# JingInAI/Quantize

Measured on AMD Instinct MI355X. Metric: quant-conv2d images/sec at batch 256 (ResNet-50, W8A8), higher is better.
Workload: dtype int8

## Files before the change

quantize_amd/capi.py:

```python
import contextlib
import ctypes
import os

from . import loader

_lib = None

QE_OK = 0
QE_ERR_UNSUPPORTED = 7
DTYPES = {"uint8": 0, "int8": 1, "int16": 2, "int32": 3, "int64": 4,
          "float16": 5, "float32": 6, "float64": 7}

ACTS = {None: 0, "none": 0, "gelu": 1}


class QeConvShape(ctypes.Structure):
    _fields_ = [(n, ctypes.c_int32) for n in ("N", "IC", "H", "W", "OC", "KH", "KW", "stride", "padding")]


class QeQParam(ctypes.Structure):
    _fields_ = [("data", ctypes.c_void_p), ("n_bits", ctypes.c_int32), ("sign", ctypes.c_int32),
                ("scale", ctypes.c_void_p), ("zero", ctypes.c_void_p), ("n_param", ctypes.c_int32)]


# ... 20 lines not shown
    "qe_tpack": (_i32, [_vp, _i32, _i64, _i32, _i32, _vp, _vp, _vp]),
    "qe_tunpack": (_i32, [_vp, _i64, _i32, _i32, _vp, _vp]),
    "qe_quantize_pack": (_i32, [_vp, _i64, _vp, _vp, _i32, _i64, _f32, _f32, _i32, _i32, _vp, _vp, _vp]),
    "qe_quantize_pack_act": (_i32, [_vp, _i64, _i32, _vp, _vp, _i32, _i64, _f32, _f32, _i32, _i32, _vp, _vp, _vp, _vp]),
    "qe_quantize_patchify": (_i32, [_vp, _i32, _i32, _i32, _i32, _i32, _vp, _vp, _i32, _f32, _f32, _i32, _i32, _vp, _vp, _vp]),
    "qe_global_avgpool": (_i32, [_vp, _i64, _i32, _vp, _vp]),
    "qe_maxpool2d_codes": (_i32, [_vp, _i32, _i32, _i32, _i32, _i32, _i32, _i32, _vp, _vp]),
    "qe_quantconv2d_path": (_i32, [_ps, _pq, _pq]),
    "qe_quantconv2d_workspace_bytes": (_sz, [_ps, _i32, _i32]),
    "qe_quantconv2d": (_i32, [_pq, _pq, _vp, _ps, _vp, _vp, _sz, _vp]),
    "qe_conv_prepared_bytes": (_sz, [_ps, _i32, _i32]),
    "qe_conv_prepared_layout": (ctypes.c_uint64, [_ps, _i32, _i32]),
    "qe_conv_prepare": (_i32, [_pq, _vp, _ps, _i32, _vp, _sz, _vp]),
    "qe_quantconv2d_prepared_workspace_bytes": (_sz, [_ps, _i32, _i32]),
    "qe_quantconv2d_prepared": (_i32, [_pq, _pq, _vp, _ps, _vp, _sz, _vp, _vp, _sz, _vp]),
    "qe_quantconv2d_requant_path": (_i32, [_ps, _pq, _pq, _pr]),
    "qe_quantconv2d_requant_workspace_bytes": (_sz, [_ps, _pq, _pq, _pr]),
    "qe_quantconv2d_requant_prepared": (_i32, [_pq, _pq, _vp, _ps, _vp, _sz, _pr, _vp, _vp, _vp, _sz, _vp]),
    "qe_quantconv2d_residual_path": (_i32, [_ps, _pq, _pq, _pr]),
    "qe_quantconv2d_residual_workspace_bytes": (_sz, [_ps, _pq, _pq, _pr]),
    "qe_quantconv2d_residual_prepared": (_i32, [_pq, _pq, _vp, _ps, _vp, _sz, _vp, _vp, _pr, _vp, _vp, _vp, _sz, _vp]),
    "qe_quantconv2d_float_input": (_i32, [_vp, _pq, _vp, _ps, _vp, _vp]),
    "qe_quantconv2d_float_input_path": (_i32, [_ps, _pq]),
    "qe_quantconv2d_float_input_workspace_bytes": (_sz, [_ps, _i32]),
    "qe_quantconv2d_float_input_ws": (_i32, [_vp, _pq, _vp, _ps, _vp, _vp, _sz, _vp]),
    "qe_conv_f32_prepare": (_i32, [_pq, _vp, _ps, _vp, _sz, _vp]),
    "qe_quantconv2d_float_input_prepared": (_i32, [_vp, _pq, _vp, _ps, _vp, _sz, _vp, _vp]),
    "qe_quantlinear": (_i32, [_pq, _pq, _vp, _i64, _i32, _i32, _vp, _vp]),
    "qe_quantlinear_path": (_i32, [_pq, _pq, _i64, _i32, _i32]),
    "qe_quantlinear_form": (_i32, [_pq, _pq, _i64, _i32, _i32, _i32]),
    "qe_quantlinear_float_input": (_i32, [_vp, _pq, _vp, _i64, _i32, _i32, _vp, _vp]),
    "qe_quantlinear_float_input_path": (_i32, [_vp, _pq, _i64, _i32, _i32]),
    "qe_quantlinear_requant_path": (_i32, [_pq, _pq, _i64, _i32, _i32, _pr, _vp]),
    "qe_quantlinear_requant_workspace_bytes": (_sz, [_pq, _pq, _i64, _i32, _i32, _pr, _vp]),
    "qe_quantlinear_requant": (_i32, [_pq, _pq, _vp, _i64, _i32, _i32, _i32, _pr, _vp, _vp, _vp, _sz, _vp]),
    "qe_quantlinear_residual_path": (_i32, [_pq, _pq, _i64, _i32, _i32]),
    "qe_quantlinear_residual_workspace_bytes": (_sz, [_pq, _pq, _i64, _i32, _i32]),
    "qe_quantlinear_residual": (_i32, [_pq, _pq, _vp, _i64, _i32, _i32, _vp, _vp, _vp, _sz, _vp]),
    "qe_quantlinear_float_input_residual_path": (_i32, [_vp, _pq, _i64, _i32, _i32]),
    "qe_quantlinear_float_input_residual_workspace_bytes": (_sz, [_vp, _pq, _i64, _i32, _i32]),
    "qe_quantlinear_float_input_residual": (_i32, [_vp, _pq, _vp, _i64, _i32, _i32, _vp, _vp, _vp, _sz, _vp]),
    "qe_layernorm_quantize_pack_path": (_i32, [_i64, _i32, _i32, _pr, _ppc]),
    "qe_layernorm_quantize_pack_workspace_bytes": (_sz, [_i64, _i32, _i32, _pr, _ppc, _vp]),
    "qe_layernorm_quantize_pack": (_i32, [_vp, _i64, _i32, _vp, _vp, _f32, _i32, _pr, _ppc, _vp, _vp, _vp, _sz, _vp]),
    "qe_attention_path": (_i32, [_i32, _i32, _i32, _i32]),
    "qe_attention": (_i32, _attn + [_vp]),
    "qe_attention_masked_path": (_i32, [_i32, _i32, _i32, _i32, _i32, _i32, _i32]),
    "qe_attention_masked": (_i32, _attn + [_vp, _i64, _i64, _vp, _i32, _vp]),
}
SYMBOLS = sorted(PROTOTYPES)
DEBUG_PROTOTYPES = {
    "qe_debug_reload_env": (None, []),
    "qe_debug_set_stamp_buffer": (None, [_vp]),
}


def lib():
    global _lib
    if _lib is not None:
        return _lib
    path = os.environ.get("QE_LIB") or loader.lib_path()
    if not os.path.exists(path):
        raise ImportError("libqe_hip.so not built: run `python -m quantize_amd.build`. No fallback exists.")
    L = ctypes.CDLL(path)
    for table in (PROTOTYPES, DEBUG_PROTOTYPES):
        for name, (restype, argtypes) in table.items():
            f = getattr(L, name)
            f.restype, f.argtypes = restype, argtypes
    _lib = L
    return L


def check(rc):
    if rc != QE_OK:
        L = lib()
        msg = L.qe_error_string(rc).decode()
        if rc == 5:
            msg += " (hipError_t %d)" % L.qe_last_hip_error()
        raise QeError(msg)


def _stream(stream=None):
    import torch
    s = torch.cuda.current_stream() if stream is None else stream
    return ctypes.c_void_p(s.cuda_stream)


def _ptr(t):
    return None if t is None else t.data_ptr()


def _ws(need, dev):
    import torch
    return torch.empty(need, dtype=torch.uint8, device=dev) if need else None


def _status(status, dev):
    import torch
    return torch.zeros(1, dtype=torch.int32, device=dev) if status is None else status


def _prep(t):
    return (t.data_ptr(), t.numel()) if t is not None and t.numel() else (None, 0)


def packed_nbytes(n, n_bits):
# ... 21 lines not shown
                           _stream(stream)))
    return out


def conv_shape(N, IC, H, W, OC, KH, KW, stride, padding):
    return QeConvShape(int(N), int(IC), int(H), int(W), int(OC), int(KH), int(KW), int(stride), int(padding))


def out_hw(sh):
    return ((sh.H + 2 * sh.padding - sh.KH) // sh.stride + 1, (sh.W + 2 * sh.padding - sh.KW) // sh.stride + 1)


def qparam(data, n_bits, sign, scale, zero):
    assert scale.numel() == zero.numel()
    q = QeQParam(data.data_ptr(), int(n_bits), 1 if sign else 0, scale.data_ptr(), zero.data_ptr(),
                 int(scale.numel()))
    q._keep = (data, scale, zero)
    return q


def workspace_bytes(sh, x_bits, w_bits):
    return int(lib().qe_quantconv2d_workspace_bytes(ctypes.byref(sh), int(x_bits), int(w_bits)))


def reload_env():
    lib().qe_debug_reload_env()


@contextlib.contextmanager
def knobs(**env):
    old = {k: os.environ.get(k) for k in env}

    def put(kv):
        for k, v in kv.items():
            if v is None:
                os.environ.pop(k, None)
            else:
                os.environ[k] = str(v)
        reload_env()

    try:
        put(env)
        yield
    finally:
        put(old)


def conv_prepared_layout(sh, x_bits, w_bits):
    return int(lib().qe_conv_prepared_layout(ctypes.byref(sh), int(x_bits), int(w_bits)))


def conv_path(sh, xq, wq):
    return int(lib().qe_quantconv2d_path(ctypes.byref(sh), ctypes.byref(xq), ctypes.byref(wq)))


def quantconv2d(xq, wq, bias, sh, out=None, workspace=None, stream=None):
    import torch
    dev = wq._keep[0].device
    OH, OW = out_hw(sh)
    if out is None:
        out = torch.empty((sh.N, sh.OC, OH, OW), dtype=torch.float32, device=dev)
    if workspace is None:
        workspace = _ws(workspace_bytes(sh, xq.n_bits, wq.n_bits), dev)
    check(lib().qe_quantconv2d(ctypes.byref(xq), ctypes.byref(wq), _ptr(bias), ctypes.byref(sh), out.data_ptr(),
                               *_prep(workspace), _stream(stream)))
    return out


def conv_prepare(wq, bias, sh, x_bits, stream=None):
    import torch
    dev = wq._keep[0].device
    need = int(lib().qe_conv_prepared_bytes(ctypes.byref(sh), int(x_bits), wq.n_bits))
    prepared = torch.empty(max(need, 0), dtype=torch.uint8, device=dev)
    check(lib().qe_conv_prepare(ctypes.byref(wq), _ptr(bias), ctypes.byref(sh), int(x_bits), *_prep(prepared), _stream(stream)))
    return prepared


def quantconv2d_prepared(xq, wq, bias, sh, prepared, out=None, workspace=None, stream=None):
    import torch
    dev = wq._keep[0].device
    OH, OW = out_hw(sh)
    if out is None:
        out = torch.empty((sh.N, sh.OC, OH, OW), dtype=torch.float32, device=dev)
    if workspace is None:
        workspace = _ws(int(lib().qe_quantconv2d_prepared_workspace_bytes(ctypes.byref(sh), xq.n_bits, wq.n_bits)), dev)
    check(lib().qe_quantconv2d_prepared(ctypes.byref(xq), ctypes.byref(wq), _ptr(bias), ctypes.byref(sh), *_prep(prepared),
                                        out.data_ptr(), *_prep(workspace), _stream(stream)))
    return out


def requant(scale, zero, qmin, qmax, n_bits, sign):
    r = QeRequant(scale.data_ptr(), zero.data_ptr(), int(scale.numel()), float(qmin), float(qmax), int(n_bits), 1 if sign else 0)
    r._keep = (scale, zero)
    return r


def requant_path(sh, xq, wq, rq):
    return int(lib().qe_quantconv2d_requant_path(ctypes.byref(sh), ctypes.byref(xq), ctypes.byref(wq), ctypes.byref(rq)))


def quantconv2d_requant_prepared(xq, wq, bias, sh, prepared, rq, out=None, status=None, workspace=None, stream=None):
    import torch
    dev = wq._keep[0].device
    OH, OW = out_hw(sh)
    if out is None:
        out = torch.empty(packed_nbytes(sh.N * sh.OC * OH * OW, rq.n_bits), dtype=torch.uint8, device=dev)
# ... 316 lines not shown
```

quantize_amd/csrc/qe_api.hip:

```cpp
#include "qe_common.h"
#include "qe_conv_plan.hpp"

#include <atomic>
#include <cstring>
#include <mutex>
#include <string>
#include <utility>
#include <vector>
#include <unistd.h>

extern char **environ;

namespace qe {

thread_local int g_last_hip_error = 0;

namespace {
struct EnvSnapshot {
    std::vector<std::pair<std::string, std::string>> kv;
};
std::atomic<EnvSnapshot *> g_env{nullptr};
std::mutex g_env_mutex;
EnvSnapshot *take_env_snapshot()
{
// ... 61 lines not shown
    if ((rc = check_qparam(x)) != QE_OK) return rc;
    if ((rc = check_qparam(w)) != QE_OK) return rc;
    return check_nparam(x, w, sh);
}

}

extern "C" const char *qe_error_string(int status)
{
    switch (status) {
        case QE_OK: return "ok";
        case QE_ERR_NBITS: return "n_bits must be in the range (0, 8]";
        case QE_ERR_RANGE: return "The input tensor is out of range.";
        case QE_ERR_DTYPE: return "unsupported element type";
        case QE_ERR_ARG: return "invalid argument";
        case QE_ERR_HIP: return "HIP runtime error";
        case QE_ERR_WORKSPACE: return "workspace too small";
        case QE_ERR_UNSUPPORTED: return "problem shape not supported by the gfx950 kernels";
        default: return "unknown error";
    }
}

extern "C" int qe_last_hip_error(void) { return qe::g_last_hip_error; }

extern "C" void qe_debug_reload_env(void)
{
    std::lock_guard<std::mutex> lock(qe::g_env_mutex);
    qe::g_env.store(qe::take_env_snapshot(), std::memory_order_release);
}
extern "C" const char *qe_version(void) { return "quantize_amd 0.1.0"; }
extern "C" const char *qe_target_arch(void) { return "gfx950"; }

namespace qe {
static ConvPlan plan_bits(const qe_conv_shape *sh, int x_bits, int w_bits)
{
    qe_qparam x{}, w{};
    x.n_bits = x_bits; x.n_param = 1;
    w.n_bits = w_bits; w.n_param = 1;
    return plan_conv({sh, &x, &w});
}
static size_t scratch_bytes(const ConvPlan &p) { return (p.m.total - p.m.prep_total + 255) / 256 * 256; }
}

extern "C" size_t qe_quantconv2d_workspace_bytes(const qe_conv_shape *shape, int x_bits, int w_bits)
{
    if (qe::check_shape(shape) != QE_OK) return 0;
    return qe::plan_bits(shape, x_bits, w_bits).m.total;
}

extern "C" int qe_quantconv2d_path(const qe_conv_shape *shape, const qe_qparam *x, const qe_qparam *w)
{
    if (qe::check_shape(shape) != QE_OK || x == nullptr || w == nullptr) return 0;
    return qe::plan_conv({shape, x, w}).route != qe::ConvRoute::Generic ? 1 : 0;
}

extern "C" int qe_quantconv2d(const qe_qparam *x, const qe_qparam *w, const float *bias,
                              const qe_conv_shape *shape, float *out,
                              void *workspace, size_t workspace_bytes, qe_stream_t stream)
{
    using namespace qe;
    const int rc = check_packed_conv(shape, x, w);
    if (rc != QE_OK) return rc;
    if (out == nullptr) return QE_ERR_ARG;
    hipStream_t s = static_cast<hipStream_t>(stream);
    const ConvPlan p = plan_conv({shape, x, w, reinterpret_cast<uintptr_t>(out)});
    if (p.route == ConvRoute::Generic) return launch_conv_generic(true, x->data, x, w, bias, shape, out, s);
    return launch_conv_mfma(p, x, w, bias, shape, out, workspace, workspace_bytes, nullptr, 0, false, s, nullptr, nullptr);
}

extern "C" size_t qe_conv_prepared_bytes(const qe_conv_shape *shape, int x_bits, int w_bits)
{
    if (qe::check_shape(shape) != QE_OK) return 0;
    return qe::plan_prepared(shape, x_bits, w_bits).prep_total;
}

extern "C" uint64_t qe_conv_prepared_layout(const qe_conv_shape *shape, int x_bits, int w_bits)
{
    if (qe::check_shape(shape) != QE_OK) return 0;
    return qe::prepared_layout(qe::plan_prepared(shape, x_bits, w_bits), shape);
}

extern "C" size_t qe_quantconv2d_prepared_workspace_bytes(const qe_conv_shape *shape, int x_bits, int w_bits)
{
    if (qe::check_shape(shape) != QE_OK) return 0;
    const qe::ConvPlan p = qe::plan_bits(shape, x_bits, w_bits);
    return p.m.total - p.m.prep_total;
}

extern "C" int qe_conv_prepare(const qe_qparam *w, const float *bias, const qe_conv_shape *shape, int x_bits,
                               void *prepared, size_t prepared_bytes, qe_stream_t stream)
{
    using namespace qe;
    int rc = check_shape(shape);
    if (rc != QE_OK) return rc;
    if ((rc = check_qparam(w)) != QE_OK) return rc;
    if ((rc = check_nparam(nullptr, w, shape)) != QE_OK) return rc;
    if (!(x_bits > 0 && x_bits <= 8)) return QE_ERR_NBITS;
    return prepare_conv_tables(plan_prepared(shape, x_bits, w->n_bits), w, bias, shape, prepared, prepared_bytes,
                               static_cast<hipStream_t>(stream));
}

extern "C" int qe_quantconv2d_prepared(const qe_qparam *x, const qe_qparam *w, const float *bias,
                                       const qe_conv_shape *shape, const void *prepared, size_t prepared_bytes,
                                       float *out, void *workspace, size_t workspace_bytes, qe_stream_t stream)
{
    using namespace qe;
// ... 301 lines not shown
```

quantize_amd/csrc/qe_conv_plan.hip:

```cpp
#include "qe_conv_plan.hpp"
#include "qe_conv_mfma_kernel.hpp"

#include <algorithm>
#include <cstdlib>

namespace qe {

static int knob(const char *name, int dflt)
{
    const char *e = env_get(name);
    return e ? atoi(e) : dflt;
}

static size_t align_up(size_t v, size_t a) { return (v + a - 1) / a * a; }

static const int kNiw[3][3] = {{7, 4, 2}, {4, 2, 1}, {2, 1, 0}};
static const int kWN[3] = {1, 2, 4};

static MfmaPlan make_plan8(const qe_conv_shape *sh, int w_bits, bool x4 = false)
{
    MfmaPlan p;
    p.OH = (sh->H + 2 * sh->padding - sh->KH) / sh->stride + 1;
    p.OW = (sh->W + 2 * sh->padding - sh->KW) / sh->stride + 1;
    p.KK = sh->KH * sh->KW;
// ... 222 lines not shown
}

MfmaPlan plan_prepared(const qe_conv_shape *sh, int x_bits, int w_bits)
{
    qe_conv_shape s1 = *sh;
    const int64_t img = (int64_t)sh->IC * sh->H * sh->W;
    s1.N = img >= 64 ? 1 : (int)((64 + img - 1) / img);
    return make_plan(&s1, x_bits, w_bits);
}

uint64_t prepared_layout(const MfmaPlan &p, const qe_conv_shape *sh)
{
    if (!p.ok || p.prep_total == 0) return 0;
    uint64_t h = 1469598103934665603ull;
    auto mix = [&](uint64_t v) { h = (h ^ v) * 1099511628211ull; };
    mix(p.smallic ? 1 : 0); mix((uint64_t)p.OCP); mix((uint64_t)p.NG); mix((uint64_t)p.KK); mix((uint64_t)sh->KH); mix((uint64_t)sh->KW);
    mix((uint64_t)sh->IC); mix((uint64_t)sh->OC); mix((uint64_t)p.prep_total); mix((uint64_t)p.ep_off); mix((uint64_t)p.ws_off);
    return h | 1ull;
}

struct PwrFit {
    int tw = 0, ks = 0, groups = 1;
    bool s2 = false;
};

static bool pwr_plan(const qe_conv_shape *sh, const qe_qparam *x, const qe_qparam *w, uintptr_t xa, PwrFit *pl)
{
    const int mode = knob("QE_PWR", 2);
    if (mode == 0) return false;
    if (sh->KH != 1 || sh->KW != 1 || sh->padding != 0 || (sh->stride != 1 && sh->stride != 2)) return false;
    if (x->n_bits != 8 || w->n_bits != 8 || x->n_param != 1) return false;
    if (sh->IC != 64 && sh->IC != 128 && sh->IC != 256) return false;
    if (sh->OC % 32 != 0 || sh->OC < 128 || sh->N < 1) return false;
    const bool s2 = sh->stride == 2;
    if (s2 && ((sh->H & 1) || (sh->W & 7) || sh->W > 64 || knob("QE_PWR_S2", 1) == 0)) return false;
    const int OH = s2 ? sh->H / 2 : sh->H, OW = s2 ? sh->W / 2 : sh->W;
    const int64_t P = (int64_t)OH * OW;
    const int tw = (P % 224 == 0) ? 224 : ((P % 196 == 0) ? 196 : 0);
    if (tw == 0) return false;
    if (s2 && (tw % OW != 0 || tw / OW > 8)) return false;
    if (mode == 1 && !s2 && P != tw) return false;
    if ((int64_t)sh->N * sh->IC * sh->H * sh->W < 16 || (int64_t)sh->OC * P >= (1ll << 29) || (int64_t)sh->IC * sh->H * sh->W >= (1ll << 31)) return false;
    if ((reinterpret_cast<uintptr_t>(w->data) & 15) != 0 || (xa & (s2 ? 7 : 3)) != 0) return false;
    if ((reinterpret_cast<uintptr_t>(w->scale) & 3) != 0) return false;
    const int ks = sh->IC / 32;
    const int waves = ks == 8 ? 8 : 4;
    if (sh->OC < 64 * waves) return false;
    const int strips = sh->OC / 32;
    const int g = knob("QE_PWR_GROUPS", 0);
    pl->tw = tw; pl->ks = ks; pl->groups = (g >= 1 && strips % g == 0) ? g : 1; pl->s2 = s2;
    return true;
}

static int pwr7_plan(const qe_conv_shape *sh, const qe_qparam *x, const qe_qparam *w, uintptr_t xa, int *groups)
{
    if (knob("QE_PWR", 2) == 0 || knob("QE_PWR7", 1) == 0) return 0;
    if (sh->KH != 1 || sh->KW != 1 || sh->stride != 1 || sh->padding != 0 || sh->H * sh->W != 49) return 0;
    if (x->n_bits != 8 || w->n_bits != 8 || x->n_param != 1) return 0;
    if (sh->IC != 128 && sh->IC != 256 && sh->IC != 512) return 0;
    const int gi = sh->IC == 512 ? 2 : 4;
    if (sh->OC % 32 != 0 || sh->OC < 512 || sh->N < gi || sh->N % gi != 0) return 0;
    if ((int64_t)sh->N * sh->IC * 49 >= (1ll << 31) || (int64_t)sh->OC * 49 >= (1ll << 29)) return 0;
    if ((reinterpret_cast<uintptr_t>(w->data) & 15) != 0 || (xa & 15) != 0) return 0;
    const int tiles = sh->N / gi, strips = sh->OC / 32;
    int g = 1;
    while (tiles * g < kNumCU && strips % (2 * g) == 0 && strips / (2 * g) >= 8) g *= 2;
    const int ge = knob("QE_PWR_GROUPS", 0);
    *groups = (ge >= 1 && strips % ge == 0) ? ge : g;
    return gi;
}

static bool flatd_plan(const qe_conv_shape *sh, const qe_qparam *x, const qe_qparam *w, uintptr_t xa)
{
    if (sh->KH != 1 || sh->KW != 1 || sh->stride != 1 || sh->padding != 0) return false;
    if (x->n_bits != 8 || w->n_bits != 8 || x->n_param != 1) return false;
    if (sh->IC % FD_CK != 0 || sh->IC < 2 * FD_CK || sh->OC < 1 || sh->N < 1) return false;
    const int64_t P = (int64_t)sh->H * sh->W;
    if ((int64_t)sh->N * sh->IC * P < 16 || (int64_t)sh->OC * P >= (1ll << 29) || (int64_t)sh->IC * P >= (1ll << 31)) return false;
    if ((reinterpret_cast<uintptr_t>(w->data) & 15) != 0) return false;
    return P == 49 && sh->OC % 4 == 0 && (xa & 15) == 0;
}

static int64_t block_map(ConvPlan &p, int64_t n_units, int per_image, int64_t per_tile, bool knob_ok = true)
{
    const int64_t per_xcd = (n_units + 7) / 8;
    const int64_t k = knob_ok ? (int64_t)knob("QE_CHUNK_IMAGES", 1 << 20) * per_image : per_xcd;
    p.chunk = (int)std::max<int64_t>(1, std::min<int64_t>(per_xcd, k));
    const int64_t runs = (n_units + p.chunk - 1) / p.chunk;
    return (runs + 7) / 8 * p.chunk * 8 * per_tile;
}

static bool plan_rq_patch(const MfmaPlan &m, const ConvRequest &r)
{
    if (m.flat || m.flatg || m.ws || m.GI != 1 || (m.OH * m.OW) % 4 != 0 || (m.TH * m.OW) % 4 != 0) return false;
    if ((r.rq_out & 3) != 0 || knob("QE_RQ_PATCH", 1) == 0) return false;
    const int wm = m.cfg == 0 ? 4 : (m.cfg == 1 ? 2 : 1);
    const int kkt = m.KK == 1 ? 1 : ((m.KK == 9 && r.sh->KW == 3) ? 9 : 0);
    if (m.sm2) return mfma_has_patch(MfKind::Sm2, wm, m.niw, kkt, m.NS);
    return mfma_has_patch(m.smallic ? MfKind::Stem : MfKind::Halo, wm, m.niw, kkt, m.NS);
}

static void plan_mfma_launch(ConvPlan &p, const ConvRequest &r, bool rq)
{
    const MfmaPlan &m = p.m;
    const qe_conv_shape *sh = &p.run;
    p.tiles_h = (m.OH + m.TH - 1) / m.TH;
    p.n_pix_tiles = ((sh->N + m.GI - 1) / m.GI) * p.tiles_h;
    p.n_oc_tiles = m.OCP / m.MT;
    if (m.flatg) {
        p.tiles_h = 1;
        p.n_pix_tiles = (sh->N + m.GI - 1) / m.GI;
    } else if (m.flat) {
        p.tiles_h = m.IHT;
        p.n_pix_tiles = sh->N * p.tiles_h;
    }
    p.blocks = block_map(p, p.n_pix_tiles, p.tiles_h, p.n_oc_tiles);
    auto clipped_lo = [](int pad, int stride, int O) { return std::min(O, (pad + stride - 1) / stride); };
    auto clipped_hi = [](int I, int pad, int K, int stride, int O) {
        const int full_last = (I + pad - K) >= 0 ? (I + pad - K) / stride : -1;
        return std::max(0, std::min(O, O - 1 - full_last));
    };
    p.n_top = clipped_lo(sh->padding, sh->stride, m.OH);
    p.n_bot = clipped_hi(sh->H, sh->padding, sh->KH, sh->stride, m.OH);
    p.n_lft = clipped_lo(sh->padding, sh->stride, m.OW);
    p.n_rgt = clipped_hi(sh->W, sh->padding, sh->KW, sh->stride, m.OW);

    if (m.flat || m.flatg) {
        p.lds = m.lds;
        if (rq) {
            p.ptab_off = (int)align_up(m.lds, 16);
            p.lds = p.ptab_off + (m.flatg ? (size_t)m.GI * m.MT * sh->H * sh->W : (size_t)m.MT * 32 * m.ni);
        }
        return;
    }
    p.rq_patch = rq && plan_rq_patch(m, r);
    const size_t stage_bytes = p.rq_patch ? std::max(m.lds, (size_t)32 * 1024) : m.lds;
    size_t lds_e = stage_bytes;
    const size_t tab = (size_t)m.MT * (sh->KH + 1) * (sh->KW + 1) * sizeof(int);
    const size_t off = align_up(stage_bytes, 16);
    if (off + tab <= (size_t)(m.sm2 ? MF_MAX_LDS_SM2 : MF_MAX_LDS)) { p.ptab_off = (int)off; lds_e = off + tab; }
    const int ncls = (1 + p.n_top + p.n_bot) * (1 + p.n_lft + p.n_rgt);
    p.ctab = p.ptab_off != 0 && p.n_top + p.n_bot < m.OH && p.n_lft + p.n_rgt < m.OW && ncls <= (sh->KH + 1) * (sh->KW + 1) &&
             knob("QE_CTAB", 1) != 0;
    const int units = m.GI * m.IHT * ((sh->W + 3) / 4);
    p.split = units <= 64 ? 4 : (units <= 128 ? 2 : 1);
    p.lds = (m.ws && !p.ctab) ? m.lds : lds_e;
}

ConvPlan plan_conv(const ConvRequest &r)
{
    ConvPlan p;
    const qe_conv_shape *sh = r.sh;
    p.OH = (sh->H + 2 * sh->padding - sh->KH) / sh->stride + 1;
    p.OW = (sh->W + 2 * sh->padding - sh->KW) / sh->stride + 1;
    if (p.OH > 0 && p.OW > 0) p.y_bytes = align_up((size_t)sh->N * sh->OC * p.OH * p.OW * sizeof(float), 256);
    p.m = make_plan(sh, r.x->n_bits, r.w->n_bits);
    const MfmaPlan &m = p.m;
    if (r.x->n_param != 1 || !m.ok) return p;
    p.run = m.sub ? dense_shape(sh) : *sh;
    const qe_conv_shape *rs = &p.run;

    qe_qparam xr = *r.x;
    uintptr_t xa = reinterpret_cast<uintptr_t>(r.x->data);
    if (m.sub_x4 || m.expand) { xr.n_bits = 8; xr.sign = 1; }
    if (m.sub || m.expand) xa = 0;
    if (m.sub_x4) {
        p.pre = PrePass::SubX4;
        p.pre_blocks = ((int64_t)sh->N * sh->IC * rs->H * ((rs->W + 7) / 8) + 255) / 256;
    } else if (m.sub) {
        const int64_t n_planes = (int64_t)sh->N * sh->IC;
        const int nq = (rs->W + 7) / 8;
        int log_nq = 0;
        while ((1 << log_nq) < nq) ++log_nq;
        const int units2 = rs->H << log_nq;
        if (sh->stride == 2 && (sh->H % 2) == 0 && (1 << log_nq) == nq && 16 * nq <= 2 * sh->W && units2 <= 256 &&
            knob("QE_SUB2", 1) != 0) {
            int log_up = 3;
            while ((1 << log_up) < units2) ++log_up;
            p.pre = PrePass::Sub2;
            p.sub2_log_nq = log_nq;
            p.sub2_log_up = log_up;
            const int ppb = (256 >> log_up) * 4;
            p.pre_blocks = (n_planes + ppb - 1) / ppb;
        } else {
            const bool wide = sh->stride == 2 && (sh->W % 4) == 0 && sh->W >= 16;
            const int units = rs->H * ((rs->W + (wide ? 7 : 3)) / (wide ? 8 : 4));
            const int ppb = units >= 1024 ? 1 : 1024 / units;
            p.pre = wide ? PrePass::SubWide : PrePass::SubNarrow;
            p.pre_blocks = (n_planes + ppb - 1) / ppb;
        }
    }
    if (p.pre_blocks > 0x7fffffffLL) return p;

    PwrFit pf;
    int g7 = 1;
    if (r.residual) {
        if (r.rq_bits != 0 && (r.rq_bits != 8 || r.rq_n_param != 1)) return p;
        if (m.sub || m.expand || rs->stride != 1) return p;
        if (pwr_plan(rs, &xr, r.w, xa, &pf)) p.route = ConvRoute::Pwr;
        else if (rs->IC == 512 && (p.pwr7_gi = pwr7_plan(rs, &xr, r.w, xa, &g7)) != 0) p.route = ConvRoute::Pwr7;
        else return p;
        p.fused = true;
    } else {
        const bool rq = r.rq_bits > 0;
        if (rq) {
            if (r.rq_bits != 8 || r.rq_n_param != 1) return p;
            if (m.flat || m.flatg) {
                const size_t patch = m.flatg ? (size_t)m.GI * m.MT * rs->H * rs->W : (size_t)m.MT * 32 * m.ni;
                if (align_up(m.lds, 16) + patch > (size_t)MF_MAX_LDS) return p;
            }
            p.fused = true;
        }
        const bool pwr_ok = rq ? (r.rq_out & 15) == 0 && knob("QE_PWR_RQ", 1) != 0 : true;
        const bool fd_ok = flatd_plan(rs, &xr, r.w, xa) && knob("QE_FLATD", 1) != 0 &&
                           (!rq || (rs->OC % 32 == 0 && (r.rq_out & 15) == 0 && knob("QE_FLATD_RQ", 1) != 0));
        if (pwr_ok && pwr_plan(rs, &xr, r.w, xa, &pf)) p.route = ConvRoute::Pwr;
        else if (pwr_ok && (rq || (r.out & 15) == 0) && (p.pwr7_gi = pwr7_plan(rs, &xr, r.w, xa, &g7)) != 0) p.route = ConvRoute::Pwr7;
        else if (fd_ok) p.route = ConvRoute::Flatd;
        else p.route = ConvRoute::Mfma;
    }

    if (p.route == ConvRoute::Pwr) {
        p.pwr_tw = pf.tw; p.pwr_ks = pf.ks; p.pwr_groups = pf.groups; p.pwr_s2 = pf.s2;
        const int64_t P = pf.s2 ? (int64_t)(rs->H / 2) * (rs->W / 2) : (int64_t)rs->H * rs->W;
        p.tiles_h = (int)(P / pf.tw);
        p.n_pix_tiles = rs->N * p.tiles_h;
        p.blocks = block_map(p, p.n_pix_tiles, p.tiles_h, pf.groups);
    } else if (p.route == ConvRoute::Pwr7) {
        p.pwr_groups = g7;
        p.tiles_h = 1;
        p.n_pix_tiles = rs->N / p.pwr7_gi;
        p.blocks = block_map(p, p.n_pix_tiles, 1, g7, false);
    } else if (p.route == ConvRoute::Flatd) {
        const char *e8 = env_get("QE_FLATD8");
        p.fd_w8 = e8 ? atoi(e8) != 0 && rs->OC > 128 : rs->OC >= 1024;
        const int MT = p.fd_w8 ? 256 : 128;
        p.n_oc_tiles = (rs->OC + MT - 1) / MT;
        p.tiles_h = 1;
        p.n_pix_tiles = (rs->N + 3) / 4;
        p.blocks = block_map(p, p.n_pix_tiles, p.tiles_h, p.n_oc_tiles);
    } else {
        plan_mfma_launch(p, r, p.fused);
    }
    if (p.blocks > 0x7fffffffLL) { p.route = ConvRoute::Generic; p.fused = false; }
    return p;
}

}
```

quantize_amd/csrc/qe_conv_pwr.hip:

```cpp
#include "qe_conv_mfma_kernel.hpp"
#include "qe_conv_plan.hpp"

#include <utility>

namespace qe {

struct PwrArgs {
    const uint8_t *x;
    const uint8_t *w;
    const float *x_scale, *x_zero, *w_scale, *w_zero, *bias;
    int x_sign, w_sign, w_per_tensor;
    float *out;
    int N, IC, OC, P;
    int tiles_per_image, n_pix_tiles, chunk;
    int n_groups;
    int strips_per_group;
    unsigned long long *dbg;
    int W_in, PIN, OW;
    uint8_t *rq_out;
    const float *rq_scale, *rq_zero;
    float rq_qmin, rq_qmax, rq_lo, rq_hi;
    unsigned rq_offset;
    int32_t *rq_status;
    const float *res;
// ... 9 lines not shown
{
#pragma unroll
    for (int k = 0; k < NB; ++k) id[k] = *reinterpret_cast<const float4 *>(a.res + e + off[k]);
}
template <bool RQ, int NB>
__device__ __forceinline__ void res_flush(const PwrArgs &a, const ResBlock<RQ, NB> &b, const uint32_t (&off)[NB])
{
    if (a.out != nullptr) {
#pragma unroll
        for (int k = 0; k < NB; ++k) *reinterpret_cast<float4 *>(a.out + b.e + off[k]) = b.v[k];
    }
    if constexpr (RQ) {
#pragma unroll
        for (int k = 0; k < NB; ++k) *reinterpret_cast<uint32_t *>(a.rq_out + b.e + off[k]) = b.pk[k];
    }
}
template <bool RQ>
__device__ __forceinline__ void res_make(const RqConst &rqc, float4 y, float4 id, float4 &out, uint32_t &pk, bool &bad)
{
    float v[4] = {y.x + id.x, y.y + id.y, y.z + id.z, y.w + id.w};
#pragma unroll
    for (int j = 0; j < 4; ++j) v[j] = (v[j] > 0.0f || v[j] != v[j]) ? v[j] : 0.0f;
    out = make_float4(v[0], v[1], v[2], v[3]);
    if constexpr (RQ) {
        pk = 0;
#pragma unroll
        for (int j = 0; j < 4; ++j) {
            bool b = false;
            const float r = rq_value(rqc, v[j], b);
            bad |= b;
            pk = __builtin_amdgcn_cvt_pk_u8_f32(r, j, pk);
        }
    }
}

template <int NT, int WAVES, int KS, int TW> struct PwrGeom {
    static constexpr int THREADS = 64 * WAVES;
    static constexpr int IC = 32 * KS;
    static constexpr int RS = 32 * NT;
    static constexpr int NTP = 32 * NT;
    static constexpr int XBYTES = IC * RS;
    static constexpr int XINSTR = XBYTES / 1024;
    static constexpr int PXW = (XINSTR + WAVES - 1) / WAVES;
    static constexpr int TAB = WAVES * 4 * 32 * 4;
    static constexpr int PATCH = 8 * TW * 4;
    static constexpr int PPR = TW / 4;
    static constexpr int NRB = (8 * PPR + 63) / 64;
    static constexpr int PPRB = (TW + 15) / 16;
    static constexpr int NRQ = (32 * PPRB + 63) / 64;
    static constexpr int LDS = XBYTES + TAB + WAVES * PATCH;
};

template <int NT, int WAVES, int KS, int TW, bool S2 = false, bool RQ = false, bool RES = false>
__global__ __launch_bounds__(64 * WAVES, 2) void conv_pwr_kernel(const PwrArgs a)
{
    using G = PwrGeom<NT, WAVES, KS, TW>;
    static_assert(!(S2 && RES), "the residual epilogue has stride-1 instances only");
    constexpr bool RQT = RQ && !RES;
    static_assert(TW % 4 == 0 && TW <= 32 * NT && TW > 32 * (NT - 1), "tile width");
    constexpr int RS = G::RS, PXW = G::PXW;
    static_assert((NT & 1) == 1, "row stride must be an odd multiple of 32 B");
    extern __shared__ __attribute__((aligned(16))) uint8_t smem[];

    const int tid = threadIdx.x, lane = tid & 63;
    const int wave = __builtin_amdgcn_readfirstlane(tid >> 6);
    const int col = lane & 31, h = lane >> 5;
    const int P = a.P;
#ifdef QE_STAMP
    unsigned long long st[8] = {0, 0, 0, 0, 0, 0, 0, 0};
    unsigned long long tprev = qe_stamp();
    const unsigned long long tstart = tprev;
#endif

    int pt, og;
    {
        const int bid = blockIdx.x;
        const int idx = bid >> 3;
        const int j = idx / a.n_groups;
        og = idx - j * a.n_groups;
        const int c = j / a.chunk;
        pt = (c * 8 + (bid & 7)) * a.chunk + (j - c * a.chunk);
    }
    if (pt >= a.n_pix_tiles) return;
    const int n0 = pt / a.tiles_per_image;
    const int p0 = (pt - n0 * a.tiles_per_image) * TW;

    uint8_t *Xs = smem;
    float *tab = reinterpret_cast<float *>(smem + G::XBYTES) + wave * 128;
    float *patch = reinterpret_cast<float *>(smem + G::XBYTES + G::TAB) + wave * (8 * TW);

    const int strip0 = og * a.strips_per_group + wave;
    const int n_my = (a.strips_per_group - wave + WAVES - 1) / WAVES;
    v4i wf[KS];
    float c_sw, c_zw, c_bi;
    auto load_w = [&](int strip) __attribute__((always_inline)) {
        const int oc = strip * 32 + col;
        const float *psw = a.w_scale + (a.w_per_tensor ? 0 : oc);
        const float *pzw = a.w_zero + (a.w_per_tensor ? 0 : oc);
        const float *pbi = a.bias ? a.bias + oc : psw;
        const uint8_t *wl = a.w + (int64_t)oc * G::IC + 16 * h;
        asm volatile("global_load_dword %0, %3, off\n\tglobal_load_dword %1, %4, off\n\tglobal_load_dword %2, %5, off"
                     : "=&v"(c_sw), "=&v"(c_zw), "=&v"(c_bi) : "v"(psw), "v"(pzw), "v"(pbi) : "memory");
#define QE_PWR_LW(K, OFF) if constexpr (KS > K) asm volatile("global_load_dwordx4 %0, %1, off offset:" #OFF : "=v"(wf[K]) : "v"(wl) : "memory")
        QE_PWR_LW(0, 0); QE_PWR_LW(1, 32); QE_PWR_LW(2, 64); QE_PWR_LW(3, 96);
        QE_PWR_LW(4, 128); QE_PWR_LW(5, 160); QE_PWR_LW(6, 192); QE_PWR_LW(7, 224);
#undef QE_PWR_LW
    };
    auto wait_w = [&](auto n_tag) __attribute__((always_inline)) {
        constexpr int N = decltype(n_tag)::value;
        if constexpr (KS == 2) asm volatile("s_waitcnt vmcnt(%5)" : "+v"(c_sw), "+v"(c_zw), "+v"(c_bi), "+v"(wf[0]), "+v"(wf[1]) : "i"(N) : "memory");
        else if constexpr (KS == 4) asm volatile("s_waitcnt vmcnt(%7)" : "+v"(c_sw), "+v"(c_zw), "+v"(c_bi), "+v"(wf[0]), "+v"(wf[1]), "+v"(wf[2]), "+v"(wf[3]) : "i"(N) : "memory");
        else asm volatile("s_waitcnt vmcnt(%11)" : "+v"(c_sw), "+v"(c_zw), "+v"(c_bi), "+v"(wf[0]), "+v"(wf[1]), "+v"(wf[2]), "+v"(wf[3]), "+v"(wf[4]), "+v"(wf[5]), "+v"(wf[6]), "+v"(wf[7]) : "i"(N) : "memory");
        if (!a.bias) c_bi = 0.0f;
    };
    if (n_my > 0) load_w(strip0);

    const int n_xi = (G::XINSTR % WAVES == 0 || wave < G::XINSTR % WAVES) ? PXW : PXW - 1;
    int fix_i = -1;
    uint32_t tail_word = 0;
    if constexpr (S2) {
        constexpr int THREADS = 64 * WAVES;
        constexpr int MAXP = 8;
        const int RT = TW / a.OW;
        const int NU = G::IC * RT;
        const int np = a.W_in >> 3;
        const int r0 = p0 / a.OW;
        const uint8_t *xin = a.x + (int64_t)n0 * G::IC * a.PIN;
        constexpr int UPT = (G::IC * 8 + THREADS - 1) / THREADS;
#pragma unroll
        for (int i0 = 0; i0 < UPT; i0 += 2) {
            uint2 d[2][MAXP];
            int cc[2], rr[2];
            bool live[2];
#pragma unroll
            for (int q = 0; q < 2; ++q) {
                const int u = tid + THREADS * (i0 + q);
                live[q] = (i0 + q) < UPT && u < NU;
                const int uc = live[q] ? u : 0;
                cc[q] = uc / RT; rr[q] = uc - cc[q] * RT;
                const uint8_t *row = xin + (int64_t)cc[q] * a.PIN + (int64_t)(2 * (r0 + rr[q])) * a.W_in;
#pragma unroll
                for (int j = 0; j < MAXP; ++j) {
                    const int jc = j < np ? j : np - 1;
                    __builtin_memcpy(&d[q][j], row + 8 * jc, 8);
                }
            }
#pragma unroll
            for (int q = 0; q < 2; ++q) {
                uint32_t *dst = reinterpret_cast<uint32_t *>(Xs + cc[q] * RS + rr[q] * a.OW);
#pragma unroll
                for (int j = 0; j < MAXP; ++j)
                    if (live[q] && j < np) dst[j] = __builtin_amdgcn_perm(d[q][j].y, d[q][j].x, 0x06040200u) ^ 0x80808080u;
            }
        }
    } else {
    const int64_t x_total = (int64_t)a.N * G::IC * P;
    const int64_t x_last16 = x_total - 16;
    tail_word = *reinterpret_cast<const uint32_t *>(a.x + x_total - 4);
#pragma unroll
    for (int i = 0; i < PXW; ++i) {
        const int e = 64 * (wave + WAVES * i) + lane;
        const int c = e / (RS / 16);
        const int j = e - c * (RS / 16);
        int64_t src = ((int64_t)n0 * G::IC + c) * P + p0 + 16 * j;
        bool skip = false;
        if (src > x_last16) {
            if (src < x_total && i < n_xi) { skip = true; fix_i = i; }
            else src = x_last16;
        }
        if (i < n_xi && !skip)
            __builtin_amdgcn_global_load_lds((const __attribute__((address_space(1))) void *)(a.x + src),
                                             (__attribute__((address_space(3))) void *)(Xs + 1024 * (wave + WAVES * i)), 16, 0, 0);
    }
// ... 618 lines not shown
#undef QE_PWR7_LAUNCH
#undef QE_PWR7_LAUNCH2
#undef QE_PWR7_LAUNCH3
}

int launch_pwr(const ConvPlan &p, const qe_qparam *x, const qe_qparam *w, const float *bias, float *out, hipStream_t s,
               const RequantHost *rq, const float *res)
{
    if (p.route == ConvRoute::Pwr7) {
        launch_pwr7(p, x, w, bias, out, s, rq, res);
        QE_LAUNCH_CHECK();
        return QE_OK;
    }
    const qe_conv_shape *sh = &p.run;
    PwrArgs a;
    a.res = res;
    rq_args(a, rq);
    a.x = static_cast<const uint8_t *>(x->data); a.w = static_cast<const uint8_t *>(w->data);
    a.x_scale = x->scale; a.x_zero = x->zero; a.w_scale = w->scale; a.w_zero = w->zero; a.bias = bias;
    a.x_sign = x->sign; a.w_sign = w->sign; a.w_per_tensor = (w->n_param == 1);
    a.out = out; a.N = sh->N; a.IC = sh->IC; a.OC = sh->OC;
    a.W_in = sh->W; a.PIN = sh->H * sh->W;
    a.OW = p.pwr_s2 ? sh->W / 2 : sh->W;
    a.P = p.pwr_s2 ? (sh->H / 2) * (sh->W / 2) : sh->H * sh->W;
    a.tiles_per_image = p.tiles_h;
    a.n_pix_tiles = p.n_pix_tiles;
    a.n_groups = p.pwr_groups;
    a.strips_per_group = sh->OC / 32 / p.pwr_groups;
    a.dbg = g_mfma_dbg;
    a.chunk = p.chunk;
    const int64_t blocks = p.blocks;
#define QE_PWR_LAUNCH2(WV, KSV, TWV, S2V, RQV)                                                                             \
    do {                                                                                                                    \
        static const bool ok_ = hipFuncSetAttribute(reinterpret_cast<const void *>(&conv_pwr_kernel<7, WV, KSV, TWV, S2V, RQV>), \
                                                    hipFuncAttributeMaxDynamicSharedMemorySize, PwrGeom<7, WV, KSV, TWV>::LDS) == hipSuccess; \
        (void)ok_;                                                                                                          \
        constexpr size_t lds_ = PwrGeom<7, WV, KSV, TWV>::LDS;                                                              \
        hipLaunchKernelGGL((conv_pwr_kernel<7, WV, KSV, TWV, S2V, RQV>), dim3((unsigned)blocks), dim3(64 * WV), lds_, s, a); \
    } while (0)
#define QE_PWR_LAUNCH1(WV, KSV, TWV, S2V) do { if (rq != nullptr) QE_PWR_LAUNCH2(WV, KSV, TWV, S2V, true); else QE_PWR_LAUNCH2(WV, KSV, TWV, S2V, false); } while (0)
#define QE_PWR_LAUNCHR(WV, KSV, TWV, RQV)                                                                                   \
    do {                                                                                                                    \
        static const bool ok_ = hipFuncSetAttribute(reinterpret_cast<const void *>(&conv_pwr_kernel<7, WV, KSV, TWV, false, RQV, true>), \
                                                    hipFuncAttributeMaxDynamicSharedMemorySize, PwrGeom<7, WV, KSV, TWV>::LDS) == hipSuccess; \
        (void)ok_;                                                                                                          \
        constexpr size_t lds_ = PwrGeom<7, WV, KSV, TWV>::LDS;                                                              \
        hipLaunchKernelGGL((conv_pwr_kernel<7, WV, KSV, TWV, false, RQV, true>), dim3((unsigned)blocks), dim3(64 * WV), lds_, s, a); \
    } while (0)
#define QE_PWR_LAUNCH(WV, KSV, TWV)                                                                                         \
    do {                                                                                                                    \
        if (res != nullptr) { if (rq != nullptr) QE_PWR_LAUNCHR(WV, KSV, TWV, true); else QE_PWR_LAUNCHR(WV, KSV, TWV, false); } \
        else if (p.pwr_s2) QE_PWR_LAUNCH1(WV, KSV, TWV, true); else QE_PWR_LAUNCH1(WV, KSV, TWV, false);                      \
    } while (0)
    if (p.pwr_tw == 224) {
        if (p.pwr_ks == 2) QE_PWR_LAUNCH(4, 2, 224); else if (p.pwr_ks == 4) QE_PWR_LAUNCH(4, 4, 224); else QE_PWR_LAUNCH(8, 8, 224);
    } else {
        if (p.pwr_ks == 2) QE_PWR_LAUNCH(4, 2, 196); else if (p.pwr_ks == 4) QE_PWR_LAUNCH(4, 4, 196); else QE_PWR_LAUNCH(8, 8, 196);
    }
#undef QE_PWR_LAUNCH1
#undef QE_PWR_LAUNCH2
#undef QE_PWR_LAUNCHR
#undef QE_PWR_LAUNCH
    QE_LAUNCH_CHECK();
    return QE_OK;
}

}
```

Baseline: 63000.

## Route 512-channel stride-2 1x1 convs to a deep-K pwr kernel, skipping subsample pass

Adds a dedicated plan and kernel instance for 1x1 stride-2 convolutions with 512 input channels at 28x28 (ResNet-50 downsample), using a 16-slice K tile with 4 waves. The kernel loads the stride-2 input directly, decimating and sign-flipping it into LDS, so the separate subsample pre-pass and its extra memory traffic are avoided. Weight-fragment loads and the wait statement are extended to 16 registers, and launch bounds drop to one block per CU for this instance. That increases register and LDS pressure and lowers occupancy. A debug route-query entry point is also added.

```diff
diff --git a/quantize_amd/capi.py b/quantize_amd/capi.py
--- a/quantize_amd/capi.py
+++ b/quantize_amd/capi.py
@@ -96,6 +96,7 @@
 DEBUG_PROTOTYPES = {
     "qe_debug_reload_env": (None, []),
     "qe_debug_set_stamp_buffer": (None, [_vp]),
+    "qe_debug_conv_route": (_i32, [_ps, _pq, _pq]),
 }
 
 
@@ -223,6 +224,16 @@
 
 def conv_path(sh, xq, wq):
     return int(lib().qe_quantconv2d_path(ctypes.byref(sh), ctypes.byref(xq), ctypes.byref(wq)))
+
+
+ROUTES = ("generic", "pwr", "pwr7", "flatd", "mfma")
+PRE_PASSES = ("none", "sub_x4", "sub2", "sub_wide", "sub_narrow")
+
+
+def conv_route(sh, xq, wq):
+    v = int(lib().qe_debug_conv_route(ctypes.byref(sh), ctypes.byref(xq), ctypes.byref(wq)))
+    assert v >= 0
+    return {"route": ROUTES[v & 15], "pre": PRE_PASSES[(v >> 4) & 15], "s2": bool(v & 256), "expand": bool(v & 512), "ks": v >> 10}
 
 
 def quantconv2d(xq, wq, bias, sh, out=None, workspace=None, stream=None):
diff --git a/quantize_amd/csrc/qe_api.hip b/quantize_amd/csrc/qe_api.hip
--- a/quantize_amd/csrc/qe_api.hip
+++ b/quantize_amd/csrc/qe_api.hip
@@ -137,6 +137,14 @@
 {
     if (qe::check_shape(shape) != QE_OK || x == nullptr || w == nullptr) return 0;
     return qe::plan_conv({shape, x, w}).route != qe::ConvRoute::Generic ? 1 : 0;
+}
+
+extern "C" int qe_debug_conv_route(const qe_conv_shape *shape, const qe_qparam *x, const qe_qparam *w)
+{
+    if (qe::check_shape(shape) != QE_OK || x == nullptr || w == nullptr) return -1;
+    const qe::ConvPlan p = qe::plan_conv({shape, x, w});
+    return (int)p.route + 16 * (int)p.pre + 256 * (p.pwr_s2 ? 1 : 0) + 512 * (p.m.expand ? 1 : 0) +
+           1024 * (p.route == qe::ConvRoute::Pwr ? p.pwr_ks : 0);
 }
 
 extern "C" int qe_quantconv2d(const qe_qparam *x, const qe_qparam *w, const float *bias,
diff --git a/quantize_amd/csrc/qe_conv_plan.hip b/quantize_amd/csrc/qe_conv_plan.hip
--- a/quantize_amd/csrc/qe_conv_plan.hip
+++ b/quantize_amd/csrc/qe_conv_plan.hip
@@ -298,6 +298,28 @@
     return true;
 }
 
+constexpr int kPwrDeepTW = 196, kPwrDeepKS = 16, kPwrDeepWaves = 4;
+constexpr size_t kPwrMaxLds = 160 * 1024;
+constexpr size_t pwr_lds_bytes(int ic, int nt, int waves, int tw)
+{
+    return (size_t)ic * 32 * nt + (size_t)waves * 4 * 32 * 4 + (size_t)waves * 8 * tw * 4;
+}
+static_assert(pwr_lds_bytes(32 * kPwrDeepKS, 7, kPwrDeepWaves, kPwrDeepTW) <= kPwrMaxLds, "the 512-channel tile fits with 4 waves");
+static_assert(pwr_lds_bytes(32 * kPwrDeepKS, 7, 8, kPwrDeepTW) > kPwrMaxLds, "... and not with 8");
+static bool pwr_s2_deep_plan(const qe_conv_shape *sh, const qe_qparam *x, const qe_qparam *w, PwrFit *pl)
+{
+    if (knob("QE_PWR", 2) == 0 || knob("QE_PWR_S2", 1) == 0 || knob("QE_PWR_S2D", 1) == 0) return false;
+    if (sh->KH != 1 || sh->KW != 1 || sh->padding != 0 || sh->stride != 2) return false;
+    if (x->n_bits != 8 || w->n_bits != 8 || x->n_param != 1) return false;
+    if (sh->IC != 32 * kPwrDeepKS || sh->H != 28 || sh->W != 28) return false;
+    if (sh->OC % 32 != 0 || sh->OC < 32 || sh->N < 1) return false;
+    if ((int64_t)sh->OC * kPwrDeepTW >= (1ll << 29)) return false;
+    if ((reinterpret_cast<uintptr_t>(w->data) & 15) != 0 || (reinterpret_cast<uintptr_t>(x->data) & 7) != 0) return false;
+    if ((reinterpret_cast<uintptr_t>(w->scale) & 3) != 0) return false;
+    pl->tw = kPwrDeepTW; pl->ks = kPwrDeepKS; pl->groups = 1; pl->s2 = true;
+    return true;
+}
+
 static int pwr7_plan(const qe_conv_shape *sh, const qe_qparam *x, const qe_qparam *w, uintptr_t xa, int *groups)
 {
     if (knob("QE_PWR", 2) == 0 || knob("QE_PWR7", 1) == 0) return 0;
@@ -403,6 +425,9 @@
     p.m = make_plan(sh, r.x->n_bits, r.w->n_bits);
     const MfmaPlan &m = p.m;
     if (r.x->n_param != 1 || !m.ok) return p;
+    PwrFit pf;
+    const bool s2_deep = m.sub && !m.sub_x4 && !m.expand && !r.residual && r.rq_bits == 0 && pwr_s2_deep_plan(sh, r.x, r.w, &pf);
+    if (s2_deep) p.m.sub = false;
     p.run = m.sub ? dense_shape(sh) : *sh;
     const qe_conv_shape *rs = &p.run;
 
@@ -438,7 +463,6 @@
     }
     if (p.pre_blocks > 0x7fffffffLL) return p;
 
-    PwrFit pf;
     int g7 = 1;
     if (r.residual) {
         if (r.rq_bits != 0 && (r.rq_bits != 8 || r.rq_n_param != 1)) return p;
@@ -460,7 +484,8 @@
         const bool pwr_ok = rq ? (r.rq_out & 15) == 0 && knob("QE_PWR_RQ", 1) != 0 : true;
         const bool fd_ok = flatd_plan(rs, &xr, r.w, xa) && knob("QE_FLATD", 1) != 0 &&
                            (!rq || (rs->OC % 32 == 0 && (r.rq_out & 15) == 0 && knob("QE_FLATD_RQ", 1) != 0));
-        if (pwr_ok && pwr_plan(rs, &xr, r.w, xa, &pf)) p.route = ConvRoute::Pwr;
+        if (s2_deep) p.route = ConvRoute::Pwr;
+        else if (pwr_ok && pwr_plan(rs, &xr, r.w, xa, &pf)) p.route = ConvRoute::Pwr;
         else if (pwr_ok && (rq || (r.out & 15) == 0) && (p.pwr7_gi = pwr7_plan(rs, &xr, r.w, xa, &g7)) != 0) p.route = ConvRoute::Pwr7;
         else if (fd_ok) p.route = ConvRoute::Flatd;
         else p.route = ConvRoute::Mfma;
diff --git a/quantize_amd/csrc/qe_conv_pwr.hip b/quantize_amd/csrc/qe_conv_pwr.hip
--- a/quantize_amd/csrc/qe_conv_pwr.hip
+++ b/quantize_amd/csrc/qe_conv_pwr.hip
@@ -85,7 +85,7 @@
 };
 
 template <int NT, int WAVES, int KS, int TW, bool S2 = false, bool RQ = false, bool RES = false>
-__global__ __launch_bounds__(64 * WAVES, 2) void conv_pwr_kernel(const PwrArgs a)
+__global__ __launch_bounds__(64 * WAVES, KS >= 16 ? 1 : 2) void conv_pwr_kernel(const PwrArgs a)
 {
     using G = PwrGeom<NT, WAVES, KS, TW>;
     static_assert(!(S2 && RES), "the residual epilogue has stride-1 instances only");
@@ -137,13 +137,18 @@
 #define QE_PWR_LW(K, OFF) if constexpr (KS > K) asm volatile("global_load_dwordx4 %0, %1, off offset:" #OFF : "=v"(wf[K]) : "v"(wl) : "memory")
         QE_PWR_LW(0, 0); QE_PWR_LW(1, 32); QE_PWR_LW(2, 64); QE_PWR_LW(3, 96);
         QE_PWR_LW(4, 128); QE_PWR_LW(5, 160); QE_PWR_LW(6, 192); QE_PWR_LW(7, 224);
+        QE_PWR_LW(8, 256); QE_PWR_LW(9, 288); QE_PWR_LW(10, 320); QE_PWR_LW(11, 352);
+        QE_PWR_LW(12, 384); QE_PWR_LW(13, 416); QE_PWR_LW(14, 448); QE_PWR_LW(15, 480);
 #undef QE_PWR_LW
     };
     auto wait_w = [&](auto n_tag) __attribute__((always_inline)) {
         constexpr int N = decltype(n_tag)::value;
         if constexpr (KS == 2) asm volatile("s_waitcnt vmcnt(%5)" : "+v"(c_sw), "+v"(c_zw), "+v"(c_bi), "+v"(wf[0]), "+v"(wf[1]) : "i"(N) : "memory");
         else if constexpr (KS == 4) asm volatile("s_waitcnt vmcnt(%7)" : "+v"(c_sw), "+v"(c_zw), "+v"(c_bi), "+v"(wf[0]), "+v"(wf[1]), "+v"(wf[2]), "+v"(wf[3]) : "i"(N) : "memory");
-        else asm volatile("s_waitcnt vmcnt(%11)" : "+v"(c_sw), "+v"(c_zw), "+v"(c_bi), "+v"(wf[0]), "+v"(wf[1]), "+v"(wf[2]), "+v"(wf[3]), "+v"(wf[4]), "+v"(wf[5]), "+v"(wf[6]), "+v"(wf[7]) : "i"(N) : "memory");
+        else if constexpr (KS == 8) asm volatile("s_waitcnt vmcnt(%11)" : "+v"(c_sw), "+v"(c_zw), "+v"(c_bi), "+v"(wf[0]), "+v"(wf[1]), "+v"(wf[2]), "+v"(wf[3]), "+v"(wf[4]), "+v"(wf[5]), "+v"(wf[6]), "+v"(wf[7]) : "i"(N) : "memory");
+        else asm volatile("s_waitcnt vmcnt(%19)" : "+v"(c_sw), "+v"(c_zw), "+v"(c_bi), "+v"(wf[0]), "+v"(wf[1]), "+v"(wf[2]), "+v"(wf[3]), "+v"(wf[4]), "+v"(wf[5]), "+v"(wf[6]), "+v"(wf[7]),
+                          "+v"(wf[KS - 8]), "+v"(wf[KS - 7]), "+v"(wf[KS - 6]), "+v"(wf[KS - 5]), "+v"(wf[KS - 4]), "+v"(wf[KS - 3]), "+v"(wf[KS - 2]), "+v"(wf[KS - 1]) : "i"(N) : "memory");
+        static_assert(KS == 2 || KS == 4 || KS == 8 || KS == 16, "the wait statement names every weight register");
         if (!a.bias) c_bi = 0.0f;
     };
     if (n_my > 0) load_w(strip0);
@@ -151,7 +156,40 @@
     const int n_xi = (G::XINSTR % WAVES == 0 || wave < G::XINSTR % WAVES) ? PXW : PXW - 1;
     int fix_i = -1;
     uint32_t tail_word = 0;
-    if constexpr (S2) {
+    if constexpr (S2 && KS == 16) {
+        constexpr int THREADS = 64 * WAVES;
+        constexpr int NU = G::IC * 7;
+        constexpr int UPT = NU / THREADS;
+        constexpr int UB = 7;
+        static_assert(TW == 196 && NU % THREADS == 0 && UPT % UB == 0, "whole units per thread");
+        const uint8_t *xin = a.x + (int64_t)n0 * G::IC * 784;
+#pragma unroll
+        for (int i0 = 0; i0 < UPT; i0 += UB) {
+            uint2 d[UB][8];
+#pragma unroll
+            for (int q = 0; q < UB; ++q) {
+                const int u = tid + THREADS * (i0 + q);
+                const int c = u / 7, rp = u - c * 7;
+                const uint8_t *row = xin + c * 784 + rp * 112;
+#pragma unroll
+                for (int j = 0; j < 8; ++j) __builtin_memcpy(&d[q][j], row + 56 * (j >> 2) + 8 * (j & 3), 8);
+            }
+#pragma unroll
+            for (int q = 0; q < UB; ++q) {
+                const int u = tid + THREADS * (i0 + q);
+                const int c = u / 7, rp = u - c * 7;
+                uint32_t e[8];
+#pragma unroll
+                for (int j = 0; j < 8; ++j) e[j] = __builtin_amdgcn_perm(d[q][j].y, d[q][j].x, 0x06040200u) ^ 0x80808080u;
+                uint32_t *dst = reinterpret_cast<uint32_t *>(Xs + c * RS + rp * 28);
+                dst[0] = e[0]; dst[1] = e[1]; dst[2] = e[2];
+                dst[3] = (e[3] & 0xffffu) | (e[4] << 16);
+                dst[4] = (e[4] >> 16) | (e[5] << 16);
+                dst[5] = (e[5] >> 16) | (e[6] << 16);
+                dst[6] = (e[6] >> 16) | (e[7] << 16);
+            }
+        }
+    } else if constexpr (S2) {
         constexpr int THREADS = 64 * WAVES;
         constexpr int MAXP = 8;
         const int RT = TW / a.OW;
@@ -876,7 +914,9 @@
         if (res != nullptr) { if (rq != nullptr) QE_PWR_LAUNCHR(WV, KSV, TWV, true); else QE_PWR_LAUNCHR(WV, KSV, TWV, false); } \
         else if (p.pwr_s2) QE_PWR_LAUNCH1(WV, KSV, TWV, true); else QE_PWR_LAUNCH1(WV, KSV, TWV, false);                      \
     } while (0)
-    if (p.pwr_tw == 224) {
+    if (p.pwr_ks == 16) {
+        QE_PWR_LAUNCH2(4, 16, 196, true, false);
+    } else if (p.pwr_tw == 224) {
         if (p.pwr_ks == 2) QE_PWR_LAUNCH(4, 2, 224); else if (p.pwr_ks == 4) QE_PWR_LAUNCH(4, 4, 224); else QE_PWR_LAUNCH(8, 8, 224);
     } else {
         if (p.pwr_ks == 2) QE_PWR_LAUNCH(4, 2, 196); else if (p.pwr_ks == 4) QE_PWR_LAUNCH(4, 4, 196); else QE_PWR_LAUNCH(8, 8, 196);
```

After: 63350, median of 2. About the same (+0.6%).
